# cqf7419/LiDAR-GS

Measured on AMD Instinct MI355X. Metric: LiDAR range-view frames/sec (fwd+bwd), higher is better.
Workload: dtype f32

## Files before the change

lidar-gs_amd/csrc/api.hip:

```cpp
#include "lidargs_common.h"
#include "../../include/lidargs_rasterizer.h"

#include <math.h>
#include <stdio.h>
#include <string.h>
#include <limits>
#include <algorithm>
#include <atomic>
#include <mutex>

namespace {
using lg::SegPlan;

thread_local char g_err[512] = "";
thread_local long long g_counters[10] = {0, 0, 0, 0, 0, 0, 0, 0, -1, -1};
thread_local int g_counters_on = 0;
struct CounterPage {
    unsigned long long* dev = nullptr; unsigned long long* host = nullptr; hipEvent_t done = nullptr; int device = -1; bool pending = false;
    bool ready() {
        int d = -1;
        if (hipGetDevice(&d) != hipSuccess) return false;
        if (dev && d == device) return true;
        if (dev) { (void)hipFree(dev); dev = nullptr; }
        if (done) { (void)hipEventDestroy(done); done = nullptr; }
// ... 151 lines not shown
    if (e == hipSuccess) e = hipEventRecord(t_host_read.copied, s);
    return (int)e;
}
int read_words_end(int n, uint32_t* out) {
    const hipError_t e = hipEventSynchronize(t_host_read.copied);
    if (e == hipSuccess) memcpy(out, t_host_read.words, (size_t)n * sizeof(uint32_t));
    return (int)e;
}

struct Profiler {
    static constexpr int MAX_CALLS = 256;
    struct Call { int n = 0; const char* names[LIDARGS_MAX_STAGES]; hipEvent_t ev[LIDARGS_MAX_STAGES + 1]; bool created = false; };
    bool enabled = false;
    int every = 1;
    int seen[2] = {0, 0};
    int ncalls = 0;
    Call* calls = nullptr;
    Call* cur = nullptr;
};
Profiler g_prof;
}

namespace lg {
int api_fail(int code, const char* msg) { return fail(code, "%s", msg); }
int api_check_launch(hipStream_t s, int debug, const char* what) { return check_launch(s, debug, what); }
std::atomic<bool> g_deterministic_seen{false};
int refuse_deterministic(const char* entry) {
    if (!deterministic_requested()) return 0;
    return fail(LIDARGS_ERR_INVALID_ARGUMENT, "%s: LIDARGS_DETERMINISTIC=1 is not supported by this entry point (only lidargs_forward / lidargs_backward are); unset it for this call", entry);
}
int api_read_words_zero_behind(const uint32_t* dev, int n, uint32_t* out, void* zero, size_t zero_bytes, hipStream_t s) {
    hipError_t e = (hipError_t)read_words_begin(dev, n, s);
    if (e == hipSuccess && zero && zero_bytes) e = hipMemsetAsync(zero, 0, zero_bytes, s);
    return e == hipSuccess ? read_words_end(n, out) : (int)e;
}
bool prune_footprints() { return !switches().no_prune; }
int tile_rows() { return switches().tile_rows ? switches().tile_rows : 4; }

FrameLayout frame_layout(int num_rendered, int W, int H, int col_lo, int col_hi, FrameVariant variant) {
    const bool surfel = variant == FRAME_SURFEL, shell = variant == FRAME_SHELL;
    FrameLayout L;
    L.TH = 4 << (num_rendered & 3);
    L.Rp = (size_t)(num_rendered & ~3);
    L.grid = make_grid(W, H, L.TH);
    if (col_lo >= 0) { L.grid.x_lo = col_lo / LG_TILE_W; L.grid.x_n = (col_hi + LG_TILE_W - 1) / LG_TILE_W - L.grid.x_lo; }
    L.patches = (size_t)L.grid.num_tiles() * L.grid.waves_per_tile;
    L.plan = surfel ? plan_segments(L.Rp, L.grid.waves_per_tile, 1) : plan_segments(L.Rp, L.grid.waves_per_tile, 0, (size_t)L.grid.window_patches());
    L.S = choose_segments(L.Rp, L.plan.max_segments);
    L.fused = L.plan.fused && !shell;
    L.gated = L.fused || (L.plan.n_rounds > 0 && L.plan.rounds[0] < L.S);
    L.flags = L.fused || L.S > 1 || shell || surfel;
    L.work_list = switches().work_lists && !surfel && !shell && work_lists_fit(L.patches, L.S) && !L.fused && L.S > 1;
    L.buf = surfel ? SURFEL_BUFFERS : GAUSS_BUFFERS;
    return L;
}
void prof_begin(hipStream_t s, int kind) {
    Profiler& p = g_prof;
    p.cur = nullptr;
    if (!p.enabled) return;
    if (p.seen[kind]++ % p.every != 0) return;
    if (!p.calls) p.calls = new Profiler::Call[Profiler::MAX_CALLS];
    p.cur = &p.calls[p.ncalls % Profiler::MAX_CALLS];
    p.ncalls++;
    if (!p.cur->created) { for (auto& e : p.cur->ev) (void)hipEventCreate(&e); p.cur->created = true; }
    p.cur->n = 0;
    (void)hipEventRecord(p.cur->ev[0], s);
}
void prof_mark(const char* name, hipStream_t s) {
    Profiler::Call* c = g_prof.cur;
    if (!c || c->n >= LIDARGS_MAX_STAGES) return;
    c->names[c->n] = name;
    (void)hipEventRecord(c->ev[c->n + 1], s);
    c->n++;
}

int bin_frame(const BinSpec& spec, const GeomView& geom, uint2* ranges, size_t P, int W, int H, int col_lo, int col_hi, bool compact,
              char* (*binning_alloc)(void*, size_t), void* binning_user, int debug, hipStream_t stream, BinnedFrame* out) {
    const bool enqueue_only = spec.capacity > 0, surfel = spec.variant == FRAME_SURFEL;
    if (!enqueue_only) LG_HIP((hipError_t)read_words_begin(geom.totals, LG_TOTALS_READ_WORDS, stream));
    RadixTail span_tail;
    span_tail.src = geom.spans; span_tail.dst = geom.span_sorted; span_tail.mode = compact ? 1 : 2;
    const uint32_t* ids_sorted = geom.id_a;
    int first_side = 1;
    const bool buckets = range_sort_buckets_ok(P);
    if (buckets) {
        launch_range_sort_buckets(geom.key_a, geom.key_b, geom.id_a, geom.id_b, P, geom.scratch, geom.totals + LG_TOTALS_KEYSPAN_WORD, span_tail, stream);
        LG_STAGE_CHECK("range sort");
    } else if (enqueue_only) {
        const int side = launch_radix_sort_pairs(geom.key_a, geom.key_b, geom.id_a, geom.id_b, P, 31, geom.scratch, stream,
                                                 switches().range_sort_bits, nullptr, SORT_MAX_RADIX_BITS, true, span_tail);
        ids_sorted = side ? geom.id_b : geom.id_a;
        LG_STAGE_CHECK("range sort");
    } else {
        first_side = launch_radix_sort_pairs(geom.key_a, geom.key_b, geom.id_a, geom.id_b, P, 8, geom.scratch, stream, 8, nullptr,
                                             SORT_MAX_RADIX_BITS, true);
        LG_STAGE_CHECK("range sort, first pass");
    }

    uint32_t totals_h[LG_TOTALS_READ_WORDS];
    if (!enqueue_only) {
        LG_HIP((hipError_t)read_words_end(LG_TOTALS_READ_WORDS, totals_h));
        if (!buckets) {
            uint32_t kinv = 0u, kmax = 0u;
            for (int slot = 0; slot < LG_INST_SLOTS; slot++) {
                kinv = std::max(kinv, totals_h[LG_TOTALS_KEYSPAN_WORD + 2 * slot]); kmax = std::max(kmax, totals_h[LG_TOTALS_KEYSPAN_WORD + 2 * slot + 1]);
            }
// ... 145 lines not shown
    pp.prune = lg::prune_footprints() ? 1 : 0;
    if (col_lo >= 0) {
        if (col_lo % LG_TILE_W || (col_hi % LG_TILE_W && col_hi != width) || col_hi <= col_lo || col_hi > width)
            return fail(LIDARGS_ERR_INVALID_ARGUMENT, "forward: a column wedge must be [multiple of 16, multiple of 16 or width)%s");
        pp.tile_x_lo = col_lo / LG_TILE_W; pp.tile_x_hi = (col_hi + LG_TILE_W - 1) / LG_TILE_W;
    }
    pp.n_valid = mode.n_valid;

    lg::launch_preprocess(pp, means3D, scales, rotations, opacities, colors_precomp, cov3D_precomp, beams, radii, radii_xy,
                          geom, &img, false, stream);
    LG_STAGE_CHECK("preprocess");
    lg::prof_mark("preprocess", stream);

    const lg::BinSpec spec = {is_shell ? lg::FRAME_SHELL : lg::FRAME_GAUSS, fixed_tile_rows, instance_capacity, mode.status_host, "forward"};
    lg::BinnedFrame bf;
    const int rendered = lg::bin_frame(spec, geom, img.ranges, (size_t)P, width, height, col_lo, col_hi, pp.compact != 0, binning_alloc, binning_user,
                                       debug, stream, &bf);
    if (rendered < 0) return rendered;
    const lg::FrameLayout& L = bf.L;
    const lg::BinView& bin = bf.bin;
    const size_t R = bf.R;

    lg::RenderFwdArgs ra;
    ra.fill.cnt = nullptr;
    ra.grid = L.grid; ra.ranges = img.ranges; ra.point_list = bin.val_a; ra.rec = geom.rec; ra.rowspan = geom.rowspan;
    ra.coltab = img.coltab; ra.rowtab = img.rowtab; ra.bg = background; ra.T_in = T_in;
    ra.final_T = img.final_T; ra.T_pass = T_out;
    ra.out_color = out_color; ra.out_depth = out_depth; ra.out_occ = out_occ;
    ra.seg = bin.seg; ra.S = L.S; ra.seg_len = L.plan.seg_len;
    ra.run_pass1 = (L.S > 1 || transmittance_pass || is_shell) ? 1 : 0;
    ra.flags = ra.run_pass1 ? bin.flags : nullptr; ra.R = L.Rp;
    ra.touched = geom.touched;
    ra.transmittance_only = transmittance_pass;
    ra.seg_lo = 0; ra.seg_hi = L.S; ra.front = 0; ra.alive = nullptr;
    int head = 0;
    if (!L.fused && !ra.run_pass1 && R) lg::launch_touch_all(geom.touched, radii, (size_t)P, stream);
    if (L.fused) {
        ra.flags = bin.flags; ra.alive = bin.alive;
        lg::launch_render_fused(ra, stream);
        LG_STAGE_CHECK("render fused");
        lg::prof_mark("render_fused", stream);
    } else {
    if (ra.run_pass1) {
        run_pass1_rounds(ra, L.plan, bin.alive, stream, transmittance_pass ? nullptr : &head);
        LG_STAGE_CHECK("render pass 1");
        lg::prof_mark("render_pass1", stream);
    }
    ra.seg_lo = head; ra.seg_hi = L.S;
    if (!transmittance_pass) {
        lg::launch_render_pass2(ra, stream);
        LG_STAGE_CHECK("render pass 2");
        lg::prof_mark("render_pass2", stream);
    }
    if (L.work_list) ra.fill = lg::work_list(bin);
    lg::launch_render_combine(ra, stream);
    LG_STAGE_CHECK("render combine");
    lg::prof_mark("render_combine", stream);
    }

    lg::RenderBwdArgs v = lg::RenderBwdArgs();
    v.walk.cnt = nullptr; v.grid = L.grid; v.ranges = img.ranges; v.seg = bin.seg; v.S = L.S; v.seg_len = L.plan.seg_len; v.R = L.Rp;
    v.alive = L.gated ? bin.alive : nullptr;
    v.flags = L.flags ? bin.flags : nullptr;
    lg::note_forward((size_t)P, R, L, geom.totals, ra.flags, geom.touched, (R != 0 && !transmittance_pass) ? &v : nullptr, stream);
    return rendered;
}

struct BackMode {
    bool is_shell = false;
    const float* behind = nullptr;
    const float* T_final_global = nullptr;
    int col_lo = -1, col_hi = -1;
};

int backward_impl(int P, int R, const float* background, int width, int height, const float* means3D,
                  const float* colors_precomp, const float* scales, float scale_modifier, const float* rotations,
                  const float* cov3D_precomp, const float* viewmatrix, const float* beams, const int* radii, char* geom_buffer,
                  char* binning_buffer, char* image_buffer, const BackMode& mode, const float* dL_dpix, const float* dL_dout_depth, const float* dL_dout_occ, float* dL_dmean2D,
                  float* dL_dconic, float* dL_dopacity, float* dL_dcolor, float* dL_ddepths, float* dL_dmean3D,
                  float* dL_dsphere_means3D, float* dL_dbasis_u1, float* dL_dbasis_u2, float* dL_dcov3D, float* dL_dscale,
                  float* dL_drot, int debug, hipStream_t stream) {
    (void)colors_precomp; (void)beams;
    const int col_lo = mode.col_lo, col_hi = mode.col_hi;
    if (P < 0 || R < 0 || width <= 0 || height <= 0) return fail(LIDARGS_ERR_INVALID_ARGUMENT, "backward: bad sizes%s");
    if (P == 0) return 0;
    if (!geom_buffer || !binning_buffer || !image_buffer) return fail(LIDARGS_ERR_STATE, "backward: missing forward buffers%s");
    if (!means3D || !viewmatrix || !radii || !dL_dpix || !dL_dout_depth || !dL_dout_occ || !dL_dmean2D ||
        !dL_dopacity || !dL_dcolor || !dL_dmean3D || !dL_dscale || !dL_drot || (cov3D_precomp && !dL_dcov3D))
        return fail(LIDARGS_ERR_INVALID_ARGUMENT, "backward: NULL required pointer%s");

    lg::GeomView geom; lg::geom_carve(geom_buffer, (size_t)P, lg::GAUSS_BUFFERS, &geom);
    const bool may_be_det = !mode.is_shell && col_lo < 0 && lg::g_deterministic_seen.load(std::memory_order_relaxed);
    const uint32_t* const det_mode = may_be_det ? geom.totals + LG_TOTALS_MODE_WORD : nullptr;
    if (col_lo >= 0 && (col_lo % LG_TILE_W || col_hi <= col_lo || col_hi > width)) return fail(LIDARGS_ERR_INVALID_ARGUMENT, "backward: bad column wedge%s");
    const lg::FrameLayout L = lg::frame_layout(R, width, height, col_lo, col_hi, mode.is_shell ? lg::FRAME_SHELL : lg::FRAME_GAUSS);
    lg::BinView bin; L.bin_carve(binning_buffer, &bin);
    lg::ImgView img; lg::img_carve(image_buffer, width, height, lg::make_grid(width, height, 4).num_tiles(), &img);
    lg::prof_begin(stream, 1);

    lg::ZeroRows zr;
    zr.add(dL_dmean2D, 4); zr.add(dL_dconic, 4); zr.add(dL_dopacity, 1); zr.add(dL_dcolor, 2); zr.add(dL_ddepths, 1); zr.add(dL_dmean3D, 3);
    zr.add(dL_dsphere_means3D, 3); zr.add(dL_dbasis_u1, 3); zr.add(dL_dbasis_u2, 3); zr.add(dL_dcov3D, 6); zr.add(dL_dscale, 3); zr.add(dL_drot, 4);
    lg::launch_zero_touched(geom.touched, reinterpret_cast<float4*>(geom.gacc), 4, (size_t)P, geom.tlist, geom.tcount, zr, stream, det_mode, geom.acc64);
    lg::prof_mark("bwd_zero", stream);

    lg::RenderBwdArgs rb;
    rb.walk.cnt = nullptr;
    rb.grid = L.grid; rb.ranges = img.ranges; rb.point_list = bin.val_a; rb.rec = geom.rec; rb.rowspan = geom.rowspan;
    rb.coltab = img.coltab; rb.rowtab = img.rowtab; rb.bg = background; rb.final_T = img.final_T;
    rb.seg = bin.seg; rb.S = L.S; rb.seg_len = L.plan.seg_len;
    rb.alive = L.gated ? bin.alive : nullptr;
    rb.flags = L.flags ? bin.flags : nullptr; rb.R = L.Rp;
    rb.T_final_global = mode.T_final_global; rb.behind = mode.behind;
    rb.dL_dpix = dL_dpix; rb.dL_ddepth = dL_dout_depth; rb.dL_docc = dL_dout_occ; rb.gacc = geom.gacc;
    if (L.work_list) rb.walk = lg::work_list(bin);
    rb.det_mode = det_mode; rb.acc64 = geom.acc64;
    lg::launch_render_backward(rb, stream);
    LG_STAGE_CHECK("render backward");
    lg::prof_mark("render_bwd", stream);

    lg::GaussBwdArgs gb;
    gb.P = P; gb.scale_modifier = scale_modifier;
    gb.view = viewmatrix;
    gb.means3D = means3D; gb.scales = scales; gb.rotations = rotations; gb.cov3D_precomp = cov3D_precomp; gb.radii = radii;
    gb.gacc = geom.gacc; gb.tlist = geom.tlist; gb.tcount = geom.tcount;
    gb.dL_dmean2D = dL_dmean2D; gb.dL_dconic = dL_dconic; gb.dL_dopacity = dL_dopacity; gb.dL_dcolor = dL_dcolor;
    gb.dL_ddepths = dL_ddepths; gb.dL_dbasis_u1 = dL_dbasis_u1; gb.dL_dbasis_u2 = dL_dbasis_u2;
    gb.dL_dsphere = dL_dsphere_means3D; gb.dL_dmean3D = dL_dmean3D; gb.dL_dcov3D = dL_dcov3D; gb.dL_dscale = dL_dscale;
    gb.dL_drot = dL_drot;
    gb.det_mode = det_mode; gb.acc64 = geom.acc64;
    lg::launch_gaussian_backward(gb, stream);
    LG_STAGE_CHECK("gaussian backward");
    lg::prof_mark("gaussian_bwd", stream);
    return 0;
}

}

extern "C" {

int lidargs_abi_version(void) { return LIDARGS_ABI_VERSION; }
const char* lidargs_last_error(void) { return g_err; }

int lidargs_forward(lidargs_alloc_fn geometry_alloc, void* geometry_user, lidargs_alloc_fn binning_alloc, void* binning_user,
                    lidargs_alloc_fn image_alloc, void* image_user, int P, int D, int M, const float* background, int width,
                    int height, const float* means3D, const float* shs, const float* colors_precomp, const float* opacities,
                    const float* scales, float scale_modifier, const float* rotations, const float* cov3D_precomp,
                    const float* viewmatrix, const float* projmatrix, const float* cam_pos, const float* beam_inclinations,
                    int prefiltered, int lidar_far, int lidar_near, float* out_color, float* out_depth, float* out_occ,
                    int* radii, int* radii_xy, int debug, void* stream) {
    (void)D; (void)M; (void)shs; (void)projmatrix; (void)cam_pos; (void)prefiltered;
    const float inf = std::numeric_limits<float>::infinity();
    FrameMode mode;
    mode.deterministic = lg::deterministic_requested();
    return forward_impl(geometry_alloc, geometry_user, binning_alloc, binning_user, image_alloc, image_user, P, background, width,
                        height, means3D, colors_precomp, opacities, scales, scale_modifier, rotations, cov3D_precomp, viewmatrix,
                        beam_inclinations, (float)lidar_near, (float)lidar_far, -inf, inf, nullptr, 0, out_color, out_depth,
                        out_occ, nullptr, radii, radii_xy, debug, (hipStream_t)stream, mode);
}

int lidargs_forward_enqueue(lidargs_alloc_fn geometry_alloc, void* geometry_user, lidargs_alloc_fn binning_alloc, void* binning_user,
                            lidargs_alloc_fn image_alloc, void* image_user, int P, int D, int M, const float* background, int width,
                            int height, const float* means3D, const float* shs, const float* colors_precomp, const float* opacities,
                            const float* scales, float scale_modifier, const float* rotations, const float* cov3D_precomp,
                            const float* viewmatrix, const float* projmatrix, const float* cam_pos, const float* beam_inclinations,
                            int prefiltered, int lidar_far, int lidar_near, float* out_color, float* out_depth, float* out_occ,
                            int* radii, int* radii_xy, int debug, int instance_capacity, int tile_rows, unsigned* status_host, void* stream) {
    (void)D; (void)M; (void)shs; (void)projmatrix; (void)cam_pos; (void)prefiltered;
// ... 479 lines not shown
```

lidar-gs_amd/csrc/binning.hip:

```cpp
#include "lidargs_common.h"

namespace lg {

__device__ __forceinline__ uint32_t wave_incl_scan(uint32_t v, int lane) {
#pragma unroll
    for (int o = 1; o < 64; o <<= 1) {
        const uint32_t n = __shfl_up(v, o);
        if (lane >= o) v += n;
    }
    return v;
}

__global__ void __launch_bounds__(256) k_scan_reduce(const uint32_t* __restrict__ in, size_t n, uint32_t* __restrict__ partial) {
    __shared__ uint32_t ws[4];
    const size_t base = (size_t)blockIdx.x * SCAN_BLOCK;
    uint32_t s = 0;
#pragma unroll
    for (int k = 0; k < 4; k++) {
        const size_t i = base + (size_t)k * 256 + threadIdx.x;
        if (i < n) s += in[i];
    }
#pragma unroll
    for (int o = 32; o > 0; o >>= 1) s += __shfl_xor(s, o);
    if ((threadIdx.x & 63) == 0) ws[threadIdx.x >> 6] = s;
// ... 1071 lines not shown
                                                     uint2* __restrict__ ranges, uint32_t tiles, uint32_t* __restrict__ zero, int n_zero, bool prezeroed) {
    const size_t i0 = ((size_t)blockIdx.x * 256 + threadIdx.x) * RANGES_ITEMS;
    if (blockIdx.x == 0) for (int q = threadIdx.x; q < n_zero; q += 256) zero[q] = 0u;
    if (R_dev) R = min(R, (size_t)*R_dev);
    if (R == 0) {
        if (blockIdx.x == 0) for (uint32_t t = threadIdx.x; t < tiles; t += 256) ranges[t] = make_uint2(0u, 0u);
        return;
    }
    if (i0 >= R) return;
    uint32_t key[RANGES_ITEMS];
    if constexpr (sizeof(KT) == 2) {
        const uint4 v = *reinterpret_cast<const uint4*>(tile_sorted + i0);
        const uint32_t w[4] = {v.x, v.y, v.z, v.w};
#pragma unroll
        for (int q = 0; q < 4; q++) { key[2 * q] = w[q] & 0xFFFFu; key[2 * q + 1] = w[q] >> 16; }
    } else {
        const uint4 v0 = *reinterpret_cast<const uint4*>(tile_sorted + i0), v1 = *reinterpret_cast<const uint4*>(tile_sorted + i0 + 4);
        key[0] = v0.x; key[1] = v0.y; key[2] = v0.z; key[3] = v0.w; key[4] = v1.x; key[5] = v1.y; key[6] = v1.z; key[7] = v1.w;
    }
    uint32_t prev = i0 ? (uint32_t)tile_sorted[i0 - 1] : 0u;
#pragma unroll
    for (int q = 0; q < RANGES_ITEMS; q++) {
        const size_t i = i0 + (size_t)q;
        if (i >= R) break;
        const uint32_t cur = key[q];
        if (i == 0) {
            if (!prezeroed) for (uint32_t t = 0; t < cur && t < tiles; t++) ranges[t] = make_uint2(0u, 0u);
            ranges[cur].x = 0;
        } else if (cur != prev) {
            ranges[prev].y = (uint32_t)i; ranges[cur].x = (uint32_t)i;
            if (!prezeroed) for (uint32_t t = prev + 1; t < cur; t++) ranges[t] = make_uint2(0u, 0u);
        }
        if (i == R - 1) {
            ranges[cur].y = (uint32_t)R;
            if (!prezeroed) for (uint32_t t = cur + 1; t < tiles; t++) ranges[t] = make_uint2(0u, 0u);
        }
        prev = cur;
    }
}

void launch_tile_ranges(const uint32_t* tile_sorted, size_t R, uint2* ranges, int tiles, hipStream_t s, const uint32_t* R_dev, bool key16,
                        uint32_t* zero, int n_zero, bool prezeroed) {
    if (!zero) n_zero = 0;
    if (R && key16) hipLaunchKernelGGL(k_tile_ranges<uint16_t>, dim3((unsigned)((R + 256 * RANGES_ITEMS - 1) / (256 * RANGES_ITEMS))), dim3(256), 0, s,
                                       reinterpret_cast<const uint16_t*>(tile_sorted), R, R_dev, ranges, (uint32_t)tiles, zero, n_zero, prezeroed);
    else if (R) hipLaunchKernelGGL(k_tile_ranges<uint32_t>, dim3((unsigned)((R + 256 * RANGES_ITEMS - 1) / (256 * RANGES_ITEMS))), dim3(256), 0, s, tile_sorted, R, R_dev,
                                   ranges, (uint32_t)tiles, zero, n_zero, prezeroed);
    else {
        hipMemsetAsync(ranges, 0, sizeof(uint2) * (size_t)tiles, s);
        if (n_zero) hipMemsetAsync(zero, 0, sizeof(uint32_t) * (size_t)n_zero, s);
    }
}

__global__ void __launch_bounds__(64) k_finish_totals(const uint32_t* __restrict__ totals, const unsigned long long* __restrict__ slots, uint32_t cap,
                                                      uint32_t* __restrict__ status) {
    const int lane = threadIdx.x;
    unsigned long long v[4];
#pragma unroll
    for (int q = 0; q < 4; q++) {
        v[q] = lane < LG_INST_SLOTS ? slots[4 * lane + q] : 0ull;
#pragma unroll
        for (int o = 32; o > 0; o >>= 1) v[q] += __shfl_xor(v[q], o);
    }
    if (lane == 0) {
        const uint32_t need = totals[0];
        status[0] = need; status[1] = need < cap ? need : cap;
        for (int q = 0; q < 3; q++) { status[2 + 2 * q] = (uint32_t)v[q]; status[3 + 2 * q] = (uint32_t)(v[q] >> 32); }
        status[8] = need > cap ? 1u : 0u; status[9] = cap;
        status[10] = (uint32_t)v[3]; status[11] = (uint32_t)(v[3] >> 32);
    }
}
void launch_finish_totals(const uint32_t* totals, const unsigned long long* slots, uint32_t cap, uint32_t* status, hipStream_t s) {
    hipLaunchKernelGGL(k_finish_totals, dim3(1), dim3(64), 0, s, totals, slots, cap, status);
}

}
```

lidar-gs_amd/csrc/lidargs_common.h:

```cpp
#pragma once
#include <hip/hip_runtime.h>
#include <stdint.h>
#include <stddef.h>
#include "switches.h"

#define LG_TILE_W 16
#define LG_WAVE_ROWS 4
#define LG_CHANNELS 2

#define LG_SEG_TPASS 0
#define LG_SEG_C0 1
#define LG_SEG_C1 2
#define LG_SEG_D 3
#define LG_SEG_TEND 4
#define LG_SEG_TBREAK 5
#define LG_SEG_LAST 6
#define LG_SEG_PLANES 7

#define LG_REGION 256

namespace lg {

struct Carver {
    char* p;
// ... 50 lines not shown
struct GeomView {
    float4* rec;
    uint32_t* rowspan;
    uint4* spans;
    uint2* span_sorted;
    uint32_t* key_a; uint32_t* key_b;
    uint32_t* id_a; uint32_t* id_b;
    uint32_t* block_off;
    uint32_t* totals;
    float* gacc;
    uint8_t* touched;
    uint8_t* tlist; uint16_t* tcount;
    uint32_t* scratch;
    size_t scratch_words;
    long long* acc64;
};

struct BufferWidths { int rec_f4, gacc_floats, seg_planes; bool work_list; };
constexpr BufferWidths GAUSS_BUFFERS = {4, 16, LG_SEG_PLANES, true};
constexpr BufferWidths SURFEL_BUFFERS = {5, 32, 16, false};

inline size_t geom_carve(char* base, size_t P, const BufferWidths& w, GeomView* v, bool det = false) {
    Carver c(base);
    GeomView g;
    g.rec = c.take<float4>((size_t)w.rec_f4 * P);
    g.rowspan = c.take<uint32_t>(P);
    g.spans = c.take<uint4>(P);
    g.span_sorted = c.take<uint2>(P);
    g.key_a = c.take<uint32_t>(P); g.key_b = c.take<uint32_t>(P);
    g.id_a = c.take<uint32_t>(P); g.id_b = c.take<uint32_t>(P);
    g.block_off = c.take<uint32_t>(scan_blocks(P) + 64);
    g.totals = c.take<uint32_t>(LG_TOTALS_WORDS);
    g.gacc = c.take<float>((size_t)w.gacc_floats * P);
    g.touched = c.take<uint8_t>(P + 64);
    g.tlist = c.take<uint8_t>(P + LG_REGION); g.tcount = c.take<uint16_t>(P / LG_REGION + 64);
    g.scratch_words = sort_scratch_words(P, SORT_MAX_RADIX_BITS) + scan_scratch_words(P);
    g.scratch = c.take<uint32_t>(g.scratch_words);
    const size_t plain = (size_t)(c.p - base) + 128;
    g.acc64 = c.take<long long>(16 * P);
    if (v) *v = g;
    return det ? (size_t)(c.p - base) + 128 : plain;
}

struct BinView {
    uint32_t* tile_a; uint32_t* tile_b;
    uint32_t* val_a; uint32_t* val_b;
    uint32_t* scratch;
    size_t scratch_words;
    float* seg;
    uint8_t* flags;
    uint8_t* alive;
    uint32_t* work;
    uint32_t work_cap;
};

__device__ __forceinline__ void rect_lidar(float p_c, float p_r, int rx, int ry, int gx, int gy, int& xmin, int& ymin, int& xmax, int& ymax) {
    xmin = min(gx, max(0, (int)((p_c - (float)rx) / 16.f)));
    xmax = min(gx, max(0, (int)((((p_c + (float)rx) + 16.f) - 1.f) / 16.f)));
    ymin = min(gy, max(0, (int)roundf(p_r - (float)ry)));
    ymax = min(gy, max(0, (int)fmaxf(roundf(p_r + (float)ry), roundf(p_r) + 1.f)));
}
__device__ __forceinline__ void rect_surfel(float p_c, float p_r, int rx, int ry, int gx, int gy, int& xmin, int& ymin, int& xmax, int& ymax) {
    xmin = min(gx, max(0, (int)((p_c - (float)rx) / 16.f)));
    xmax = min(gx, max(0, (int)((((p_c + (float)rx) + 16.f) - 1.f) / 16.f)));
    ymin = min(gy, max(0, (int)(p_r - (float)ry)));
    ymax = min(gy, max(0, (int)roundf(p_r + (float)ry)));
}

#define LG_WORK_REGIONS 64
#define LG_WORK_CNT_STRIDE 32
struct WorkList {
    uint32_t* cnt;
    uint32_t* items;
    uint32_t cap;
};
inline uint32_t work_cap(size_t patches, int S) { return (uint32_t)(((patches + LG_WORK_REGIONS - 1) / LG_WORK_REGIONS) * (size_t)S); }
inline size_t work_words(size_t patches, int S) { return (size_t)LG_WORK_REGIONS * (LG_WORK_CNT_STRIDE + (size_t)work_cap(patches, S)); }
inline bool work_lists_fit(size_t patches, int S) { return S <= 255 && patches < ((size_t)1 << 24); }

#define LG_SEG_LEN_DEFAULT 128
inline int choose_segments(size_t R, int max_segments) {
    if (R == 0) return 1;
    return max_segments < 1 ? 1 : max_segments;
}

inline size_t bin_carve(char* base, size_t R, size_t patches, int waves_per_tile, int S, const BufferWidths& w, BinView* v) {
    Carver c(base);
    BinView b;
    size_t n = R ? R : 1;
    b.tile_a = c.take<uint32_t>(n); b.tile_b = c.take<uint32_t>(n);
    b.val_a = c.take<uint32_t>(n); b.val_b = c.take<uint32_t>(n);
    b.scratch_words = sort_scratch_words(n);
    b.scratch = c.take<uint32_t>(b.scratch_words);
    b.seg = c.take<float>(patches * (size_t)S * w.seg_planes * 64);
    b.flags = c.take<uint8_t>((size_t)waves_per_tile * n + 64);
    b.alive = c.take<uint8_t>(patches + 64);
    b.work_cap = w.work_list ? work_cap(patches, S) : 0;
    b.work = w.work_list ? c.take<uint32_t>(work_words(patches, S)) : nullptr;
    if (v) *v = b;
    return (size_t)(c.p - base) + 128;
}

inline WorkList work_list(const BinView& b) {
    WorkList w;
    w.cnt = b.work;
    w.items = b.work + (size_t)LG_WORK_REGIONS * LG_WORK_CNT_STRIDE;
    w.cap = b.work_cap;
    return w;
}

struct ImgView {
    float* final_T;
    float* T_pass;
    uint2* ranges;
    float2* coltab;
    float2* rowtab;
};

inline size_t img_carve(char* base, int W, int H, int tiles, ImgView* v) {
    Carver c(base);
    ImgView m;
    size_t N = (size_t)W * H;
    m.final_T = c.take<float>(N);
    m.T_pass = c.take<float>(N);
    m.ranges = c.take<uint2>(tiles);
    m.coltab = c.take<float2>(W);
    m.rowtab = c.take<float2>(H);
    if (v) *v = m;
    return (size_t)(c.p - base) + 128;
}

struct TileGrid {
    int W, H, TH;
    int tiles_x, tiles_y;
    int ref_tiles_x;
    int waves_per_tile;
    int x_lo, x_n;
    __host__ __device__ int num_tiles() const { return tiles_x * tiles_y; }
    __host__ __device__ int window_patches() const { return x_n * tiles_y * waves_per_tile; }
    __host__ __device__ int global_patch(int lp) const {
        if (x_n == tiles_x) return lp;
        const int lt = lp / waves_per_tile, sub = lp - lt * waves_per_tile;
        const int ty = lt / x_n, tx = x_lo + (lt - ty * x_n);
        return (ty * tiles_x + tx) * waves_per_tile + sub;
    }
};

inline TileGrid make_grid(int W, int H, int TH) {
    TileGrid g;
    g.W = W; g.H = H; g.TH = TH;
    g.tiles_x = (W + LG_TILE_W - 1) / LG_TILE_W;
    g.tiles_y = (H + TH - 1) / TH;
    g.ref_tiles_x = g.tiles_x;
    g.waves_per_tile = TH / LG_WAVE_ROWS;
    g.x_lo = 0; g.x_n = g.tiles_x;
    return g;
}

struct PreprocessParams {
    int P, W, H, TH, tiles_x, tiles_y;
    float scale_modifier;
    float near_f, far_f;
    float shell_lo, shell_hi;
    int tile_x_lo, tile_x_hi;
    int compact;
    int prune;
    float col_step;
    float inv_col_step;
    float tan_col_step;
    const float* view;
    const uint32_t* n_valid = nullptr;
};

#ifdef LG_LANE_STATS
void lane_stats_read(unsigned long long* out, int reset);
#endif
int api_fail(int code, const char* msg);
int api_check_launch(hipStream_t s, int debug, const char* what);
int refuse_deterministic(const char* entry);
int api_read_words_zero_behind(const uint32_t* dev, int n, uint32_t* out, void* zero, size_t zero_bytes, hipStream_t s);
int tile_rows();
bool prune_footprints();
void prof_begin(hipStream_t s, int kind);
void prof_mark(const char* name, hipStream_t s);

struct SegPlan { int seg_len, max_segments, n_rounds, rounds[8]; int head; int fused; };
enum FrameVariant { FRAME_GAUSS, FRAME_SHELL, FRAME_SURFEL };
struct FrameLayout {
    int TH; size_t Rp;
    TileGrid grid;
    size_t patches; SegPlan plan; int S;
    bool fused;
    bool gated, flags, work_list;
    BufferWidths buf;
    size_t bin_carve(char* base, BinView* v) const { return lg::bin_carve(base, Rp, patches, grid.waves_per_tile, S, buf, v); }
};
FrameLayout frame_layout(int num_rendered, int W, int H, int col_lo, int col_hi, FrameVariant variant);

struct BinSpec {
    FrameVariant variant;
    int tile_rows;
    long long capacity;
    unsigned* status_host;
    const char* what;
};
struct BinnedFrame { FrameLayout L; BinView bin; size_t R; };
int bin_frame(const BinSpec& spec, const GeomView& geom, uint2* ranges, size_t P, int W, int H, int col_lo, int col_hi, bool compact,
              char* (*binning_alloc)(void*, size_t), void* binning_user, int debug, hipStream_t s, BinnedFrame* out);
struct ZeroRows { static constexpr int MAX = 12; float* p[MAX]; int w[MAX]; int n = 0;
                  void add(float* q, int width) { if (q && n < MAX) { p[n] = q; w[n] = width; n++; } } };
void launch_zero_touched(const uint8_t* touched, float4* acc, int line_f4, size_t P, uint8_t* tlist, uint16_t* tcount, const ZeroRows& zr, hipStream_t s,
                         const uint32_t* det_mode = nullptr, long long* acc64 = nullptr);
void launch_touch_all(uint8_t* touched, const int* radii, size_t P, hipStream_t s);

void launch_setup_tables(const float* beams, int W, int H, ImgView img, hipStream_t s);
void launch_preprocess(const PreprocessParams& pp, const float* means3D, const float* scales, const float* rotations,
                       const float* opacities, const float* colors, const float* cov3D_precomp, const float* beams,
                       int* radii, int* radii_xy, GeomView g, const ImgView* tables, bool filter_only, hipStream_t s);
void launch_mark_visible(int P, const float* means3D, const float* view, unsigned char* present, hipStream_t s);
void launch_debug_rects(int n, int surfel, const float* p_cr, const int* r_xy, int gx, int gy, int* rects, hipStream_t s);

void launch_exclusive_scan(const uint32_t* in, uint32_t* out, size_t n, uint32_t* total_out, uint32_t* scratch, hipStream_t s);
struct RadixTail { const void* src = nullptr; void* dst = nullptr; int mode = 0; };
struct KeyBias { uint32_t kmin, cull; const uint32_t* lin_span = nullptr; };
struct RangeSortRest { KeyBias bias; int end_bit, max_bits; };
inline RangeSortRest range_sort_rest(uint32_t kinv, uint32_t kmax) {
    RangeSortRest r;
    r.bias.kmin = (~kinv) & ~255u;
    if (kmax < r.bias.kmin) { r.bias.kmin = 0u; kmax = 0u; }
    r.bias.cull = ((kmax - r.bias.kmin) | 255u) + 1u;
    r.end_bit = 32 - __builtin_clz(r.bias.cull | 1u);
    if (r.end_bit < 9) r.end_bit = 9;
    r.max_bits = r.end_bit > 26 ? 8 : 9;
    return r;
}
int launch_radix_sort_pairs(uint32_t* key_a, uint32_t* key_b, uint32_t* val_a, uint32_t* val_b, size_t n, int end_bit,
                            uint32_t* scratch, hipStream_t s, int max_bits = 0, const uint32_t* n_dev = nullptr, int scratch_bits = 0,
                            bool vals_are_positions = false,
                            RadixTail tail = RadixTail(), int begin_bit = 0, const KeyBias* bias = nullptr);
void launch_finish_totals(const uint32_t* totals, const unsigned long long* slots, uint32_t cap, uint32_t* status, hipStream_t s);
void launch_instance_offsets(const void* span_sorted, bool compact, int TH, uint32_t* block_off, uint32_t* total_out, size_t P, hipStream_t s, bool scan = true);
void launch_emit_instances(const uint32_t* ids_sorted, const uint32_t* block_off, const void* span_sorted, bool compact, size_t P, TileGrid grid,
                           uint32_t* inst_tile, uint32_t* inst_val, hipStream_t s, uint32_t cap = 0xFFFFFFFFu, bool key16 = false,
                           uint2* ranges = nullptr,
                           bool sums_unscanned = false);
void launch_tile_ranges(const uint32_t* tile_sorted, size_t R, uint2* ranges, int tiles, hipStream_t s, const uint32_t* R_dev = nullptr, bool key16 = false,
                        uint32_t* zero = nullptr, int n_zero = 0, bool prezeroed = false);
int launch_radix_sort_pairs16(uint16_t* key_a, uint16_t* key_b, uint32_t* val_a, uint32_t* val_b, size_t n, int end_bit, uint32_t* scratch, hipStream_t s,
                              const uint32_t* n_dev = nullptr);
int radix_sort_result_side(size_t n, int end_bit);
bool range_sort_buckets_ok(size_t P);
void launch_range_sort_buckets(uint32_t* key_a, uint32_t* key_b, uint32_t* id_a, uint32_t* id_b, size_t P, uint32_t* scratch, const uint32_t* key_span,
                               RadixTail tail, hipStream_t s);

#ifdef __HIPCC__
#ifdef LG_XCD_CHUNK
__device__ __forceinline__ bool block_patch_segment(unsigned b, int patches, int S, int& patch, int& seg) {
    const unsigned stride = (unsigned)S | 1u, per = (unsigned)LG_XCD_CHUNK * stride;
    const unsigned xcd = b & 7u, j = b >> 3, c = j / per, o = j - c * per;
    patch = (int)((c * 8u + xcd) * (unsigned)LG_XCD_CHUNK + o / stride);
    seg = (int)(o % stride);
    return patch < patches && seg < S;
}
inline unsigned segment_grid(int patches, int S) {
    const unsigned group = 8u * (unsigned)LG_XCD_CHUNK;
    return (((unsigned)patches + group - 1u) / group) * group * ((unsigned)S | 1u);
}
#else
__device__ __forceinline__ bool block_patch_segment(unsigned b, int patches, int S, int& patch, int& seg) {
    const unsigned stride = (unsigned)S | 1u;
    seg = (int)(b % stride);
    patch = (int)(b / stride);
#if defined(LG_PATCH_ORDER) && LG_PATCH_ORDER == 1
    patch = patches - 1 - patch;
    return patch >= 0 && seg < S;
#elif defined(LG_PATCH_ORDER) && LG_PATCH_ORDER == 2
    seg = (int)(b / (unsigned)patches); patch = (int)(b % (unsigned)patches);
    return seg < S;
#endif
    return patch < patches && seg < S;
}
inline unsigned segment_grid(int patches, int S) { return (unsigned)patches * ((unsigned)S | 1u); }
#endif


__device__ __forceinline__ int segment_count(uint2 range, int S, int seg_len) {
    const uint32_t L = range.y - range.x;
    const uint32_t want = (L + (uint32_t)seg_len - 1u) / (uint32_t)seg_len;
    return (int)min((uint32_t)S, max(1u, want));
}
__device__ __forceinline__ uint2 segment_range(uint2 range, int St, int seg) {
    const uint32_t L = range.y - range.x;
    const uint32_t len = (L + (uint32_t)St - 1u) / (uint32_t)St;
    const uint32_t a = min(range.y, range.x + (uint32_t)seg * len);
    const uint32_t b = min(range.y, a + len);
    return make_uint2(a, b);
}

#endif

// ... 171 lines not shown
```

lidar-gs_amd/csrc/render.hip:

```cpp
#include "lidargs_common.h"
#ifdef LG_PRECISE_EXP
#define LG_EXPF(x) expf(x)
#else
#define LG_EXPF(x) __expf(x)
#endif

namespace lg {

#define LG_CHUNK 64

#ifdef LG_LANE_STATS
__device__ unsigned long long lg_lane_stats[16];
__device__ __forceinline__ void lane_stat(int base, unsigned long long m) {
    if (threadIdx.x % 64 == 0) {
        const int rows = ((m & 0xFFFFull) != 0) + ((m & 0xFFFF0000ull) != 0) + ((m & 0xFFFF00000000ull) != 0) + ((m >> 48) != 0);
        atomicAdd(&lg_lane_stats[base], 1ull); atomicAdd(&lg_lane_stats[base + 1], (unsigned long long)__popcll(m));
        atomicAdd(&lg_lane_stats[base + 2], (unsigned long long)rows); atomicAdd(&lg_lane_stats[base + 3], m ? 1ull : 0ull);
    }
}
void lane_stats_read(unsigned long long* out, int reset) {
    (void)hipMemcpyFromSymbol(out, HIP_SYMBOL(lg_lane_stats), sizeof(unsigned long long) * 16);
    if (reset) { unsigned long long z[16] = {0}; (void)hipMemcpyToSymbol(HIP_SYMBOL(lg_lane_stats), z, sizeof z); }
}
#define LG_LANE_STAT(base, m) lane_stat(base, m)
// ... 642 lines not shown
    const size_t stride = LG_SEG_PLANES * 64;
    float T = 1.f;
    const int kf = min(a.front, St);
    for (int k = 0; k < kf && T >= 0.0001f; k++) T *= sb[k * stride + LG_SEG_TPASS * 64];
    const unsigned long long open = __ballot(inside && T >= 0.0001f);
    if (lane == 0) a.alive[patch] = (St > a.front && open != 0ull) ? 255 : (uint8_t)min(a.front, 254);
}

__global__ void __launch_bounds__(64) k_render_combine(const RenderFwdArgs a) {
    const int lane = threadIdx.x;
    const int S = a.S;
    const int patch = a.grid.global_patch(blockIdx.x);
    const int wpt = a.grid.waves_per_tile;
    const int tile = patch / wpt, sub = patch - tile * wpt;
    const TileGrid& g = a.grid;
    const int x = (tile % g.tiles_x) * LG_TILE_W + (lane & 15);
    const int y = (tile / g.tiles_x) * g.TH + sub * LG_WAVE_ROWS + (lane >> 4);
    if (x >= g.W || y >= g.H) return;
    const int pix = y * g.W + x;
    const float* sb = a.seg + (size_t)patch * S * (LG_SEG_PLANES * 64) + lane;
    const size_t stride = LG_SEG_PLANES * 64;
    int St = segment_count(a.ranges[tile], S, a.seg_len);
    if (a.alive) St = min(St, (int)a.alive[patch]);

    if (a.transmittance_only) {
        float T = 1.f;
        for (int k = 0; k < St && T >= 0.0001f; k++) T *= sb[k * stride + LG_SEG_TPASS * 64];
        if (a.T_pass) a.T_pass[pix] = T;
        return;
    }
    float C0 = 0.f, C1 = 0.f, D = 0.f;
    float T_final = a.T_in ? a.T_in[pix] : 1.f, T_hand = T_final;
    bool stopped = false;
    int taken = 0, kend = 0;
    for (int k0 = 0; k0 < St; k0 += 4) {
        float c0[4], c1[4], dd[4], te[4], tb[4];
#pragma unroll
        for (int i = 0; i < 4; i++) {
            const int k = min(k0 + i, St - 1);
            c0[i] = sb[k * stride + LG_SEG_C0 * 64]; c1[i] = sb[k * stride + LG_SEG_C1 * 64]; dd[i] = sb[k * stride + LG_SEG_D * 64];
            te[i] = sb[k * stride + LG_SEG_TEND * 64]; tb[i] = sb[k * stride + LG_SEG_TBREAK * 64];
        }
#pragma unroll
        for (int i = 0; i < 4; i++) {
            const bool use = !stopped && (k0 + i < St);
            C0 += use ? c0[i] : 0.f; C1 += use ? c1[i] : 0.f; D += use ? dd[i] : 0.f;
            T_final = use ? te[i] : T_final; T_hand = use ? tb[i] : T_hand;
            taken += use ? 1 : 0;
            stopped = stopped || (use && tb[i] < 0.0001f);
        }
        kend = min(St, k0 + 4);
        if (__ballot(!stopped) == 0ull) break;
    }
    if (a.fill.cnt) {
        int n = 0;
        for (int k = kend; k > kend - 4 && k > 0 && n == 0; k--) if (__ballot(taken >= k) != 0ull) n = k;
        if (n > 0) {
            const unsigned long long act = __ballot(true);
            const int leader = __ffsll((long long)act) - 1;
            const uint32_t r = (uint32_t)patch % LG_WORK_REGIONS;
            uint32_t base = 0;
            if (lane == leader) base = atomicAdd(a.fill.cnt + r * LG_WORK_CNT_STRIDE, (uint32_t)n);
            base = (uint32_t)__shfl((int)base, leader);
            const int rank = __popcll(act & ((1ull << lane) - 1ull)), nact = __popcll(act);
            for (int k = rank; k < n; k += nact) a.fill.items[(size_t)r * a.fill.cap + base + (uint32_t)k] = ((uint32_t)patch << 8) | (uint32_t)k;
        }
    }
    const size_t N = (size_t)g.W * g.H;
    a.final_T[pix] = T_final;
    if (a.T_end_out) a.T_end_out[pix] = T_final;
    if (a.T_pass) a.T_pass[pix] = T_hand;
    const float b0 = a.bg ? a.bg[0] : 0.f, b1 = a.bg ? a.bg[1] : 0.f;
    a.out_color[pix] = C0 + T_final * b0;
    a.out_color[N + pix] = C1 + T_final * b1;
    a.out_depth[pix] = D;
    a.out_occ[pix] = 1.f - T_final;
}

static int walk2() { return switches().walk2; }
void launch_render_fused(const RenderFwdArgs& a_, hipStream_t s) {
    RenderFwdArgs a = a_; a.walk2 = walk2() & 1;
    const int waves = switches().fused_waves;
    const unsigned patches = (unsigned)a.grid.window_patches();
    if (waves == 4) hipLaunchKernelGGL(k_render_fused<4>, dim3(patches), dim3(256), 0, s, a);
    else if (waves == 16) hipLaunchKernelGGL(k_render_fused<16>, dim3(patches), dim3(1024), 0, s, a);
    else hipLaunchKernelGGL(k_render_fused<8>, dim3(patches), dim3(512), 0, s, a);
}
void launch_render_alive(const RenderFwdArgs& a, hipStream_t s) {
    const unsigned patches = (unsigned)a.grid.window_patches();
    hipLaunchKernelGGL(k_render_alive, dim3(patches), dim3(64), 0, s, a);
}
void launch_render_pass1(const RenderFwdArgs& a, hipStream_t s) {
    const unsigned blocks = segment_grid(a.grid.window_patches(), a.seg_hi - a.seg_lo);
    if (walk2() & 1) hipLaunchKernelGGL((k_render_forward<true, true>), dim3(blocks), dim3(64), 0, s, a);
    else hipLaunchKernelGGL((k_render_forward<true, false>), dim3(blocks), dim3(64), 0, s, a);
}
static int pass2_group(int seg_len) {
    return switches().p2_group ? switches().p2_group : (seg_len >= LG_SEG_LEN_DEFAULT ? 8 : 1);
}
void launch_render_pass2(const RenderFwdArgs& a, hipStream_t s) {
    const int G = pass2_group(a.seg_len);
    if (G <= 1 || a.seg_hi != a.S) {
        const unsigned blocks = segment_grid(a.grid.window_patches(), a.seg_hi - a.seg_lo);
        if (walk2() & 2) hipLaunchKernelGGL((k_render_forward<false, true>), dim3(blocks), dim3(64), 0, s, a);
        else hipLaunchKernelGGL((k_render_forward<false, false>), dim3(blocks), dim3(64), 0, s, a);
        return;
    }
// ... 13 lines not shown

__device__ __forceinline__ float xchg_xor1(float x) {
    return __int_as_float(__builtin_amdgcn_update_dpp(0, __float_as_int(x), 0xB1, 0xF, 0xF, true));
}
__device__ __forceinline__ float xchg_xor2(float x) {
    return __int_as_float(__builtin_amdgcn_update_dpp(0, __float_as_int(x), 0x4E, 0xF, 0xF, true));
}
template <int XORMASK>
__device__ __forceinline__ float xchg_swz(float x) {
    return __int_as_float(__builtin_amdgcn_ds_swizzle(__float_as_int(x), (XORMASK << 10) | 0x1F));
}

__device__ __forceinline__ float reduce_scatter16(float (&v)[16], int lane) {
#pragma unroll
    for (int k = 0; k < 8; k++) v[k] = fold_halves32(v[k], v[k + 8]);
#pragma unroll
    for (int k = 0; k < 4; k++) v[k] = fold_halves16(v[k], v[k + 4]);
    {
        const bool hi = lane & 1;
#pragma unroll
        for (int k = 0; k < 2; k++) {
            const float keep = hi ? v[k + 2] : v[k], send = hi ? v[k] : v[k + 2];
            v[k] = keep + xchg_xor1(send);
        }
    }
    {
        const bool hi = lane & 2;
        const float keep = hi ? v[1] : v[0], send = hi ? v[0] : v[1];
        v[0] = keep + xchg_xor2(send);
    }
    v[0] += __int_as_float(__builtin_amdgcn_update_dpp(0, __float_as_int(v[0]), 0x124, 0xF, 0xF, true));
    v[0] += __int_as_float(__builtin_amdgcn_update_dpp(0, __float_as_int(v[0]), 0x128, 0xF, 0xF, true));
    return v[0];
}

enum { BWD_PLAIN = 0, BWD_FIRST = 1, BWD_SECOND = 2 };
template <bool V2, int MODE>
__device__ __forceinline__ void backward_walk(const RenderBwdArgs& a, const unsigned bid, const bool det) {
    constexpr bool SECOND = MODE == BWD_SECOND;
    constexpr int OFS = V2 ? 2 : 0;
    __shared__ float4 s_rec_[4 * (LG_CHUNK + OFS)];
    __shared__ float4 s_oprow_[LG_CHUNK + OFS];
    __shared__ uint32_t s_gid_[LG_CHUNK + OFS];
    __shared__ uint32_t s_top_[SECOND ? 16 * (LG_CHUNK + OFS) : 1];
    constexpr int CS = LG_CHUNK + OFS;
    float4* const s_rec = s_rec_ + OFS;
    float4* const s_oprow = s_oprow_ + OFS;
    uint32_t* const s_gid = s_gid_ + OFS;
    uint32_t* const s_top = s_top_ + (SECOND ? 16 * OFS : 0);
    const int lane = threadIdx.x;
    const int S = a.S;
    const int wpt = a.grid.waves_per_tile;
    int patch, seg;
    if (a.walk.cnt) {
        const unsigned r = bid % LG_WORK_REGIONS, i = bid / LG_WORK_REGIONS;
        if (i >= a.walk.cnt[r * LG_WORK_CNT_STRIDE]) return;
        const uint32_t it = a.walk.items[(size_t)r * a.walk.cap + i];
        patch = (int)(it >> 8); seg = (int)(it & 255u);
    } else {
        if (!block_patch_segment(bid, a.grid.window_patches(), S, patch, seg)) return;
        patch = a.grid.global_patch(patch);
    }
    const int tile = patch / wpt, sub = patch - tile * wpt;
    const size_t stride = LG_SEG_PLANES * 64;
    const float* sb = a.seg + (size_t)patch * S * stride + lane;
    const uint2 tr = a.ranges[tile];
    const int limit = a.alive ? (int)a.alive[patch] : 255;
    const uint32_t n_lane = reinterpret_cast<const uint32_t*>(sb)[(size_t)seg * stride + LG_SEG_LAST * 64];
    const int St = segment_count(tr, S, a.seg_len);
    if (seg >= St) return;
    if (seg >= limit) return;
    uint32_t n_max = n_lane;
#pragma unroll
    for (int o = 32; o > 0; o >>= 1) n_max = max(n_max, (uint32_t)__shfl_xor((int)n_max, o));
    if (n_max == 0) return;

    const uint2 sr = segment_range(tr, St, seg);
    const int c_last = (int)((n_max - 1) / LG_CHUNK);
    const uint8_t* fl = a.flags ? a.flags + (size_t)sub * a.R + sr.x : nullptr;
    uint32_t g_first = 0u; bool have_first = false;
    if (V2) {
        const uint32_t k = (uint32_t)c_last * LG_CHUNK + lane;
        const bool in = k < n_max;
        g_first = in ? a.point_list[sr.x + k] : 0u;
        have_first = in && (!fl || fl[k] != 0);
    }
    const PixelSetup px = pixel_setup(a.grid, a.coltab, a.rowtab, tile, sub, lane);
    const size_t N = (size_t)a.grid.W * a.grid.H;

    float T = sb[(size_t)seg * stride + LG_SEG_TEND * 64];
    const float T_final = px.inside ? (a.T_final_global ? a.T_final_global[px.pix] : a.final_T[px.pix]) : 0.f;
    float g0 = 0.f, g1 = 0.f, gd = 0.f, go = 0.f;
    if (px.inside) { g0 = a.dL_dpix[px.pix]; g1 = a.dL_dpix[N + px.pix]; gd = a.dL_ddepth[px.pix]; go = a.dL_docc[px.pix]; }
    const float bgdot = a.bg ? (a.bg[0] * g0 + a.bg[1] * g1) : 0.f;
    Staged st; uint32_t gid = 0u; bool have = false;
    if (V2) { have = have_first; gid = have ? g_first : 0u; st = gather_record(a.rec, a.rowspan, g_first, have); }
    v2f acc01 = v2f{0.f, 0.f}, accdo = v2f{0.f, 0.f};
    const v2f g01 = v2f{g0, g1}, gdo = v2f{gd, go};
    {
        float b0 = 0.f, b1 = 0.f, bd = 0.f;
        const int Send = a.alive ? min(St, (int)a.alive[patch]) : St;
        {
            float acc[3] = {0.f, 0.f, 0.f};
            const int planes[3] = {LG_SEG_C0, LG_SEG_C1, LG_SEG_D};
            plane_sums<3>(acc, sb + (size_t)(seg + 1) * stride, stride, planes, Send - (seg + 1));
            b0 = acc[0]; b1 = acc[1]; bd = acc[2];
        }
// ... 225 lines not shown
```

Baseline: 1534.

## Build patch-major backward work list via prefix scan instead of atomics

```diff
diff --git a/lidar-gs_amd/csrc/api.hip b/lidar-gs_amd/csrc/api.hip
--- a/lidar-gs_amd/csrc/api.hip
+++ b/lidar-gs_amd/csrc/api.hip
@@ -227,6 +227,7 @@
     L.flags = L.fused || L.S > 1 || shell || surfel;
     L.work_list = switches().work_lists && !surfel && !shell && work_lists_fit(L.patches, L.S) && !L.fused && L.S > 1;
     L.buf = surfel ? SURFEL_BUFFERS : GAUSS_BUFFERS;
+    L.patch_major = L.work_list && col_lo < 0 && L.plan.seg_len < LG_SEG_LEN_DEFAULT;
     return L;
 }
 void prof_begin(hipStream_t s, int kind) {
@@ -478,7 +479,7 @@
         LG_STAGE_CHECK("render pass 2");
         lg::prof_mark("render_pass2", stream);
     }
-    if (L.work_list) ra.fill = lg::work_list(bin);
+    if (L.work_list) ra.fill = L.patch_major ? lg::work_list_patch_major(bin) : lg::work_list(bin);
     lg::launch_render_combine(ra, stream);
     LG_STAGE_CHECK("render combine");
     lg::prof_mark("render_combine", stream);
@@ -528,6 +529,7 @@
     zr.add(dL_dmean2D, 4); zr.add(dL_dconic, 4); zr.add(dL_dopacity, 1); zr.add(dL_dcolor, 2); zr.add(dL_ddepths, 1); zr.add(dL_dmean3D, 3);
     zr.add(dL_dsphere_means3D, 3); zr.add(dL_dbasis_u1, 3); zr.add(dL_dbasis_u2, 3); zr.add(dL_dcov3D, 6); zr.add(dL_dscale, 3); zr.add(dL_drot, 4);
     lg::launch_zero_touched(geom.touched, reinterpret_cast<float4*>(geom.gacc), 4, (size_t)P, geom.tlist, geom.tcount, zr, stream, det_mode, geom.acc64);
+    if (L.patch_major) lg::launch_work_items((int)L.patches, lg::work_list_patch_major(bin), stream);
     lg::prof_mark("bwd_zero", stream);
 
     lg::RenderBwdArgs rb;
@@ -539,7 +541,7 @@
     rb.flags = L.flags ? bin.flags : nullptr; rb.R = L.Rp;
     rb.T_final_global = mode.T_final_global; rb.behind = mode.behind;
     rb.dL_dpix = dL_dpix; rb.dL_ddepth = dL_dout_depth; rb.dL_docc = dL_dout_occ; rb.gacc = geom.gacc;
-    if (L.work_list) rb.walk = lg::work_list(bin);
+    if (L.work_list) rb.walk = L.patch_major ? lg::work_list_patch_major(bin) : lg::work_list(bin);
     rb.det_mode = det_mode; rb.acc64 = geom.acc64;
     lg::launch_render_backward(rb, stream);
     LG_STAGE_CHECK("render backward");
diff --git a/lidar-gs_amd/csrc/binning.hip b/lidar-gs_amd/csrc/binning.hip
--- a/lidar-gs_amd/csrc/binning.hip
+++ b/lidar-gs_amd/csrc/binning.hip
@@ -1147,6 +1147,50 @@
     }
 }
 
+constexpr int WORK_PATCHES = 32, WORK_THREADS = 256;
+__global__ void __launch_bounds__(WORK_THREADS) k_work_items(const uint8_t* __restrict__ walked, int patches, uint32_t* __restrict__ cnt,
+                                                            uint32_t* __restrict__ items, uint32_t room) {
+    __shared__ uint32_t s_wave[WORK_THREADS / 64];
+    __shared__ uint32_t s_n[WORK_PATCHES], s_base[WORK_PATCHES];
+    const int tid = threadIdx.x, lane = tid & 63, w = tid >> 6;
+    const int first = (int)blockIdx.x * WORK_PATCHES;
+    uint32_t front = 0u;
+    const uint32_t* const walked4 = reinterpret_cast<const uint32_t*>(walked);
+    for (int q = tid; q < first / 4; q += WORK_THREADS) {
+        const uint32_t v = walked4[q];
+        front += (v & 255u) + ((v >> 8) & 255u) + ((v >> 16) & 255u) + (v >> 24);
+    }
+#pragma unroll
+    for (int o = 32; o > 0; o >>= 1) front += __shfl_xor(front, o);
+    if (lane == 0) s_wave[w] = front;
+    __syncthreads();
+    if (w == 0) {
+        front = 0u;
+        for (int v = 0; v < WORK_THREADS / 64; v++) front += s_wave[v];
+        const int p = first + lane;
+        const uint32_t n = (lane < WORK_PATCHES && p < patches) ? walked[p] : 0u;
+        uint32_t incl = n;
+#pragma unroll
+        for (int o = 1; o < WORK_PATCHES; o <<= 1) {
+            const uint32_t up = __shfl_up(incl, o);
+            if (lane >= o) incl += up;
+        }
+        if (lane < WORK_PATCHES) { s_n[lane] = n; s_base[lane] = front + incl - n; }
+        if (lane < WORK_PATCHES && p == patches - 1) *cnt = min(front + incl, room);
+    }
+    __syncthreads();
+    for (int q = w; q < WORK_PATCHES && first + q < patches; q += WORK_THREADS / 64) {
+        const uint32_t n = s_n[q], base = s_base[q], item = (uint32_t)(first + q) << 8;
+        for (uint32_t k = (uint32_t)lane; k < n; k += 64u)
+            if (base + k < room) items[base + k] = item | k;
+    }
+}
+void launch_work_items(int patches, WorkList w, hipStream_t s) {
+    if (patches <= 0 || !w.walked) return;
+    hipLaunchKernelGGL(k_work_items, dim3((unsigned)((patches + WORK_PATCHES - 1) / WORK_PATCHES)), dim3(WORK_THREADS), 0, s,
+                       (const uint8_t*)w.walked, patches, w.cnt, w.items, (uint32_t)LG_WORK_REGIONS * w.cap);
+}
+
 __global__ void __launch_bounds__(64) k_finish_totals(const uint32_t* __restrict__ totals, const unsigned long long* __restrict__ slots, uint32_t cap,
                                                       uint32_t* __restrict__ status) {
     const int lane = threadIdx.x;
diff --git a/lidar-gs_amd/csrc/lidargs_common.h b/lidar-gs_amd/csrc/lidargs_common.h
--- a/lidar-gs_amd/csrc/lidargs_common.h
+++ b/lidar-gs_amd/csrc/lidargs_common.h
@@ -126,6 +126,7 @@
     uint8_t* alive;
     uint32_t* work;
     uint32_t work_cap;
+    uint8_t* walked;
 };
 
 __device__ __forceinline__ void rect_lidar(float p_c, float p_r, int rx, int ry, int gx, int gy, int& xmin, int& ymin, int& xmax, int& ymax) {
@@ -147,9 +148,11 @@
     uint32_t* cnt;
     uint32_t* items;
     uint32_t cap;
+    uint8_t* walked = nullptr;
 };
 inline uint32_t work_cap(size_t patches, int S) { return (uint32_t)(((patches + LG_WORK_REGIONS - 1) / LG_WORK_REGIONS) * (size_t)S); }
 inline size_t work_words(size_t patches, int S) { return (size_t)LG_WORK_REGIONS * (LG_WORK_CNT_STRIDE + (size_t)work_cap(patches, S)); }
+inline size_t walked_words(size_t patches) { return (patches + 3) / 4 + 16; }
 inline bool work_lists_fit(size_t patches, int S) { return S <= 255 && patches < ((size_t)1 << 24); }
 
 #define LG_SEG_LEN_DEFAULT 128
@@ -171,6 +174,7 @@
     b.alive = c.take<uint8_t>(patches + 64);
     b.work_cap = w.work_list ? work_cap(patches, S) : 0;
     b.work = w.work_list ? c.take<uint32_t>(work_words(patches, S)) : nullptr;
+    b.walked = w.work_list ? reinterpret_cast<uint8_t*>(c.take<uint32_t>(walked_words(patches))) : nullptr;
     if (v) *v = b;
     return (size_t)(c.p - base) + 128;
 }
@@ -182,6 +186,7 @@
     w.cap = b.work_cap;
     return w;
 }
+inline WorkList work_list_patch_major(const BinView& b) { WorkList w = work_list(b); w.walked = b.walked; return w; }
 
 struct ImgView {
     float* final_T;
@@ -266,6 +271,7 @@
     size_t patches; SegPlan plan; int S;
     bool fused;
     bool gated, flags, work_list;
+    bool patch_major;
     BufferWidths buf;
     size_t bin_carve(char* base, BinView* v) const { return lg::bin_carve(base, Rp, patches, grid.waves_per_tile, S, buf, v); }
 };
@@ -320,6 +326,7 @@
                            bool sums_unscanned = false);
 void launch_tile_ranges(const uint32_t* tile_sorted, size_t R, uint2* ranges, int tiles, hipStream_t s, const uint32_t* R_dev = nullptr, bool key16 = false,
                         uint32_t* zero = nullptr, int n_zero = 0, bool prezeroed = false);
+void launch_work_items(int patches, WorkList w, hipStream_t s);
 int launch_radix_sort_pairs16(uint16_t* key_a, uint16_t* key_b, uint32_t* val_a, uint32_t* val_b, size_t n, int end_bit, uint32_t* scratch, hipStream_t s,
                               const uint32_t* n_dev = nullptr);
 int radix_sort_result_side(size_t n, int end_bit);
diff --git a/lidar-gs_amd/csrc/render.hip b/lidar-gs_amd/csrc/render.hip
--- a/lidar-gs_amd/csrc/render.hip
+++ b/lidar-gs_amd/csrc/render.hip
@@ -718,7 +718,11 @@
         kend = min(St, k0 + 4);
         if (__ballot(!stopped) == 0ull) break;
     }
-    if (a.fill.cnt) {
+    if (a.fill.walked) {
+        int n = 0;
+        for (int k = kend; k > kend - 4 && k > 0 && n == 0; k--) if (__ballot(taken >= k) != 0ull) n = k;
+        if (lane == __ffsll((long long)__ballot(true)) - 1) a.fill.walked[patch] = (uint8_t)n;
+    } else if (a.fill.cnt) {
         int n = 0;
         for (int k = kend; k > kend - 4 && k > 0 && n == 0; k--) if (__ballot(taken >= k) != 0ull) n = k;
         if (n > 0) {
@@ -838,7 +842,11 @@
     const int S = a.S;
     const int wpt = a.grid.waves_per_tile;
     int patch, seg;
-    if (a.walk.cnt) {
+    if (a.walk.walked) {
+        if (bid >= a.walk.cnt[0]) return;
+        const uint32_t it = a.walk.items[bid];
+        patch = (int)(it >> 8); seg = (int)(it & 255u);
+    } else if (a.walk.cnt) {
         const unsigned r = bid % LG_WORK_REGIONS, i = bid / LG_WORK_REGIONS;
         if (i >= a.walk.cnt[r * LG_WORK_CNT_STRIDE]) return;
         const uint32_t it = a.walk.items[(size_t)r * a.walk.cap + i];
```

Result: faster. 1560, median of 6 (+1.7%).
